# feixh/VISMA

Measured on AMD Instinct MI355X. Metric: icp_iterations_per_sec, higher is better.
Workload: dtype f32; 1 GPU; C4 S-surf 262144->4194304, 4040 ICP iterations of a fresh registration from T=I (cold pass + warm passes), median of 1; ns=262144, nt=4194304, solver=kabsch, nn=grid, search=exact, parallelism=1 GPU, ONE persistent launch per host loop

## Files before the change

### visma_amd/csrc/grid_coop.hip

```cpp
#include <cstdlib>

#include "device_common.h"
#include "grid_coop_probe.h"

namespace visma {

namespace {

struct P12 { float x, y, z; };
#ifndef VISMA_COOP_RU
#define VISMA_COOP_RU 0
#endif
#ifndef VISMA_COOP_CAP
#define VISMA_COOP_CAP (VISMA_COOP_RU ? 344 : 352)
#endif
constexpr bool kCoopRu = VISMA_COOP_RU != 0;
constexpr int kCoopCap = VISMA_COOP_CAP;
#ifndef VISMA_COOP_DEPTH
#define VISMA_COOP_DEPTH 7
#endif
constexpr int kCoopDepth = VISMA_COOP_DEPTH;
#ifndef VISMA_COOP_ROOM
#define VISMA_COOP_ROOM 0.04f
#endif
// ... 7 lines not shown
                 "s_nop 1\n\t"
                 "v_min_f32_dpp %0, %0, %0 quad_perm:[2,3,0,1] row_mask:0xf bank_mask:0xf\n\t"
                 "s_nop 1\n\t"
                 "v_min_f32_dpp %0, %0, %0 row_half_mirror row_mask:0xf bank_mask:0xf"
                 : "=&v"(r)
                 : "v"(d));
    return r;
}

__device__ __forceinline__ unsigned pack_sec(float sec, float third, unsigned lane)
{
    if constexpr (!kCoopRu) return __float_as_uint(sec);
    return (__float_as_uint(sec) & 0xFFFF0000u) | (((__float_as_uint(third) >> 18) & 0x1FFFu) << 3) | (lane & 7u);
}
__device__ __forceinline__ float sec_of(unsigned w) { return __uint_as_float(kCoopRu ? (w & 0xFFFF0000u) : w); }
[[maybe_unused]] __device__ __forceinline__ float third_of(unsigned w) { return __uint_as_float(((w >> 3) & 0x1FFFu) << 18); }

__device__ __forceinline__ unsigned wave_scan_incl(unsigned v, int)
{
    v += (unsigned)__builtin_amdgcn_update_dpp(0, (int)v, 0x111, 0xf, 0xf, false);
    v += (unsigned)__builtin_amdgcn_update_dpp(0, (int)v, 0x112, 0xf, 0xf, false);
    v += (unsigned)__builtin_amdgcn_update_dpp(0, (int)v, 0x114, 0xf, 0xf, false);
    v += (unsigned)__builtin_amdgcn_update_dpp(0, (int)v, 0x118, 0xf, 0xf, false);
    v += (unsigned)__builtin_amdgcn_update_dpp(0, (int)v, 0x142, 0xa, 0xf, false);
    v += (unsigned)__builtin_amdgcn_update_dpp(0, (int)v, 0x143, 0xc, 0xf, false);
    return v;
}

}

struct CoopRes {
    double (*q64)[3];
    float *idx;
    float *lb;
    float *lb3;
    int first;
    double sx, sy, sz;
    int have_src;
};

template <int NTH>
__device__ __forceinline__ void coop_query_range(int ns, int bpp, int lb, int tid, int &vb, int &per_group, long long &i_begin,
                                                 long long &i_end)
{
    vb = lb;
    if ((bpp & 7) == 0) vb = (lb & 7) * (bpp >> 3) + (lb >> 3);
    const int total_groups = bpp * NTH;
    per_group = (ns + total_groups - 1) / total_groups;
    const int gid = vb * NTH + tid;
    i_begin = (long long)gid * per_group;
    i_end = i_begin + per_group < ns ? i_begin + per_group : ns;
}

template <bool PLANE, bool ONE, int NTH, bool PERSIST = false>
__device__ __forceinline__ bool coop_body(
    int ns, const float *__restrict__ s12f, const unsigned *__restrict__ start, GridParams g,
    const float4 *__restrict__ nrm, Xform64 T64, Offset64 off, float r2f, int *__restrict__ idx_out,
    float *__restrict__ d2_out, double *__restrict__ partials, unsigned long long *__restrict__ cand_count,
    const DevIcpState *__restrict__ st, int bpp, long long out_stride, const ProbDesc *__restrict__ descs,
    int nprob, const Pt64 *__restrict__ src64, const Pt64 *__restrict__ sorted64,
    const Pt64 *__restrict__ nrm64, const FoldArgs &fold, double *__restrict__ d64_out,
    Pt64 *__restrict__ wst_io, int warm, Xform64 Tprev, Pt64 *__restrict__ ru_io, unsigned *work_out = nullptr,
    const CoopRes res = CoopRes{})
{
    constexpr int NACC = Acc<PLANE>::N;
    const P12 *s12 = reinterpret_cast<const P12 *>(s12f);
    int prob, lb;
    long long row0;
    if (descs) {
        if (warm & kWarmMap) {
            prob = reinterpret_cast<const int *>(descs + nprob)[blockIdx.x];
        } else {
            int lo = 0, hi = nprob - 1;
            while (lo < hi) {
                const int mid = (lo + hi + 1) >> 1;
                if (descs[mid].first_block <= (int)blockIdx.x) lo = mid; else hi = mid - 1;
            }
            prob = lo;
        }
        const ProbDesc d = descs[prob];
        lb = (int)blockIdx.x - d.first_block;
        bpp = d.nblocks;
        src64 += d.src_off;
        ns = d.ns;
        s12 += d.sorted_off;
        sorted64 += d.sorted_off;
        if constexpr (PLANE) {
            if (nrm) nrm += d.sorted_off;
            if (nrm64) nrm64 += d.sorted_off;
        }
        row0 = d.first_block;
        start += d.start_off;
        g = d.g;
        out_stride = 0;
        idx_out += d.out_off;
        d2_out += d.out_off;
        wst_io += d.out_off;
        if (ru_io) ru_io += d.out_off;
    } else {
        prob = blockIdx.x / bpp;
        lb = blockIdx.x - prob * bpp;
        row0 = (long long)prob * bpp;
    }
    if (st) st += prob;
    {
        Xform32 T32_unused;
        if (!load_loop_state(st, T32_unused, T64, off, r2f)) return false;
        if (st) {
            warm &= ~kWarmTprev;
            if (st->have_prev && !(warm & kWarmNoCert)) {
                warm |= kWarmTprev;
#pragma unroll
                for (int k = 0; k < 12; k++) Tprev.m[k] = st->Tc_prev[k];
            }
        }
        if (!(warm & kWarmRead)) warm &= ~kWarmTprev;
    }
    const double r2d = (double)r2f;
    COOP_PROBE_BEGIN();
    idx_out += (long long)prob * out_stride;
    d2_out += (long long)prob * out_stride;
    wst_io += (long long)prob * out_stride;
    if (ru_io) ru_io += (long long)prob * out_stride;
    double acc[NACC];
#pragma unroll
    for (int a = 0; a < NACC; a++) acc[a] = 0.0;

    const int tid = thread_number<PERSIST, NTH>(), lane = tid & 63, wave = tid >> 6;
    const int oct = lane >> 3, l8 = lane & 7;
    constexpr int NW = NTH / 64;
    constexpr unsigned kCapAll = (unsigned)(NW * kCoopCap);
    int vb, per_group;
    long long i_begin, i_end;
    coop_query_range<NTH>(ns, bpp, lb, tid, vb, per_group, i_begin, i_end);

    __shared__ float4 s_qp[NTH];
    __shared__ uint2 s_item[kCapAll];
    __shared__ unsigned s_sec[kCapAll];
    __shared__ double s_p64[NTH][3];
    __shared__ double s_q64_own[PERSIST ? 1 : NTH][3];
    __shared__ float s_dprev_own[PERSIST ? 1 : NTH];
    double (*s_q64)[3] = s_q64_own;
    float *s_dprev = s_dprev_own;
    if constexpr (PERSIST) { s_q64 = res.q64; s_dprev = res.idx; }
    __shared__ unsigned short s_home[NTH];
    __shared__ unsigned s_need[NW];
    __shared__ unsigned s_m[NW];
    __shared__ unsigned short s_queue[NW][64];

    auto emit = [&](long long i, unsigned ht, bool cert, double bd, unsigned bidx, bool found, double qx, double qy, double qz,
                    float lb_new) {
        if constexpr (PERSIST) {
            res.lb[ht] = lb_new;
            return;
        }
        const unsigned long long lbw = (unsigned long long)__float_as_uint(lb_new) << 32;
        idx_out[i] = found ? (int)bidx : -1;
        if (cert) {
            reinterpret_cast<unsigned *>(&wst_io[i].w)[1] = __float_as_uint(lb_new);
        } else {
            Pt64 o8;
            o8.x = o8.y = o8.z = __longlong_as_double(-1ll);
            o8.w = 0xFFFFFFFFull | lbw;
            if (found) { o8.x = qx; o8.y = qy; o8.z = qz; o8.w = (unsigned long long)bidx | lbw; }
            wst_io[i] = o8;
        }
        d2_out[i] = (float)bd;
        if (d64_out) d64_out[i] = bd;
    };
    auto emit_ru = [&](long long i, unsigned ht, bool have, double ux, double uy, double uz, unsigned uidx, float lb3) {
        if constexpr (kCoopRu) {
            if (!ru_io) return;
            Pt64 o8;
            o8.x = o8.y = o8.z = __longlong_as_double(-1ll);
            o8.w = ~0ull;
            if (have) { o8.x = ux; o8.y = uy; o8.z = uz; o8.w = (unsigned long long)uidx | ((unsigned long long)__float_as_uint(lb3) << 32); }
            ru_io[i] = o8;
            if constexpr (PERSIST) res.lb3[ht] = have ? lb3 : __uint_as_float(0xFFFFFFFFu);
        }
    };
    auto query_p = [&](unsigned h, double (&out)[3]) { out[0] = s_p64[h][0]; out[1] = s_p64[h][1]; out[2] = s_p64[h][2]; };
    auto moments = [&](double pxd, double pyd, double pzd, unsigned bidx, double qx, double qy, double qz) {
        double nx = 0.0, ny = 0.0, nz = 0.0;
        if (PLANE) {
            if (nrm64) { const Pt64 n8 = nrm64[bidx]; nx = n8.x; ny = n8.y; nz = n8.z; }
            else { const float4 n4 = nrm[bidx]; nx = n4.x; ny = n4.y; nz = n4.z; }
        }
        accumulate_pq_d<PLANE>(acc, pxd, pyd, pzd, qx, qy, qz, nx, ny, nz, off);
    };
    auto list_rows = [&](const float px, const float py, const float pz, const float E, const float bound0, const bool want,
                         unsigned (&xb)[9], unsigned (&xe)[9], float &lbgeo2, unsigned &looked) {
        const int cx = cell_coord(px, g.mn[0], g.inv_h, g.dim[0]);
        const int cy = cell_coord(py, g.mn[1], g.inv_hs, g.dim[1]);
        const int cz = cell_coord(pz, g.mn[2], g.inv_hs, g.dim[2]);
        const int x0 = max(cx - 1, 0), x1 = min(cx + 1, g.dim[0] - 1);
        const int span = x1 + 1 - x0;
        typedef unsigned u4a __attribute__((ext_vector_type(4), aligned(4)));
        const bool yok[3] = {cy - 1 >= 0 && cy - 1 < g.dim[1], cy >= 0 && cy < g.dim[1], cy + 1 >= 0 && cy + 1 < g.dim[1]};
        const bool zok[3] = {cz - 1 >= 0 && cz - 1 < g.dim[2], cz >= 0 && cz < g.dim[2], cz + 1 >= 0 && cz + 1 < g.dim[2]};
        const int row_c = (cz * g.dim[1] + cy) * g.dim[0] + x0, pitch_y = g.dim[0], pitch_z = g.dim[1] * g.dim[0];
// ... 152 lines not shown
            if (has_w) {
                const double dx = w8.x - hp[0], dy = w8.y - hp[1], dz = w8.z - hp[2];
                double d = dx * dx;
                d += dy * dy;
                d += dz * dz;
                d2w = d;
                cert = active && t > 0.f && d < r2d && d < (double)t * (double)t * (1.0 - 1e-6);
            } else {
                cert = active && widx == 0xFFFFFFFFu && t > tlim * (1.0f + 1e-6f);
            }
            if (cert) emit(i, (unsigned)tid, true, has_w ? d2w : r2d, widx, has_w, w8.x, w8.y, w8.z, t);
            if constexpr (kCoopRu) {
                const bool has_u = u8.x == u8.x;
                float lb3 = __uint_as_float((unsigned)(u8.w >> 32));
                if constexpr (PERSIST) { if (!res.first) lb3 = res.lb3[tid]; }
                const float t3 = (lb3 - del) * (1.0f - 2.4e-7f);
                if (ru_io && active && has_w && has_u) {
                    if (cert) {
                        if constexpr (PERSIST) res.lb3[tid] = t3;
                        else reinterpret_cast<unsigned *>(&ru_io[i].w)[1] = __float_as_uint(t3);
                    } else if (lb_old > 0.f && t3 > 0.f) {
                        const unsigned uidx = (unsigned)u8.w;
                        const double dx = u8.x - hp[0], dy = u8.y - hp[1], dz = u8.z - hp[2];
                        double d2u = dx * dx;
                        d2u += dy * dy;
                        d2u += dz * dz;
                        const bool u_wins = d2u < d2w || (d2u == d2w && uidx < widx);
                        const double dm = u_wins ? d2u : d2w, dother = u_wins ? d2w : d2u;
                        if (dm < r2d && dm < (double)t3 * (double)t3 * (1.0 - 1e-6)) {
                            cert = true;
                            const float lbn = fminf(t3, sqrtf((float)dother) * (1.0f - 1e-6f));
                            if (u_wins) {
                                const Pt64 ow = w8;
                                w8.x = u8.x; w8.y = u8.y; w8.z = u8.z;
                                w8.w = (unsigned long long)uidx | ((unsigned long long)__float_as_uint(lbn) << 32);
                                widx = uidx;
                                emit_ru(i, (unsigned)tid, true, ow.x, ow.y, ow.z, (unsigned)ow.w, t3);
                                if constexpr (!PERSIST) wst_io[i] = w8;
                            } else {
                                if constexpr (PERSIST) res.lb3[tid] = t3;
                                else reinterpret_cast<unsigned *>(&ru_io[i].w)[1] = __float_as_uint(t3);
                            }
                            emit(i, (unsigned)tid, true, dm, widx, true, w8.x, w8.y, w8.z, lbn);
                        }
                    }
                } else if (ru_io && active && cert) {
                    if constexpr (PERSIST) res.lb3[tid] = __uint_as_float(0xFFFFFFFFu);
                }
            }
        }
        const bool need = active && !cert;
        const bool cfound = cert && has_w;
        s_p64[tid][0] = hp[0]; s_p64[tid][1] = hp[1]; s_p64[tid][2] = hp[2];
        if (need) {
            const float dp = sqdist_f32(make_float4((float)w8.x, (float)w8.y, (float)w8.z, 0.f), (float)hp[0], (float)hp[1], (float)hp[2]);
            const float sq = sqrtf(dp) + kCoopRoom * sqrtf(r2f);
            s_dprev[tid] = sq * sq;
        } else {
            s_q64[tid][0] = w8.x; s_q64[tid][1] = w8.y; s_q64[tid][2] = w8.z;
            s_dprev[tid] = __uint_as_float(cfound ? widx : 0xFFFFFFFFu);
        }
        if (cand_count) {
            const unsigned cc = (unsigned)__builtin_popcountll(__builtin_amdgcn_ballot_w64(cert));
            if (lane == 0 && cc) atomicAdd(cand_count + 2 * 4096 + (blockIdx.x & 4095), (unsigned long long)cc);
        }
        const unsigned long long needers = __builtin_amdgcn_ballot_w64(need);
        const unsigned rank = (unsigned)__builtin_popcountll(needers & ((1ull << lane) - 1ull));
        if (need) s_queue[wave][rank] = (unsigned short)tid;
        if (lane == 0) s_need[wave] = (unsigned)__builtin_popcountll(needers);
        COOP_MARK(9);
        __syncthreads();
        COOP_MARK(10);
        set_phase_prio(1);
        unsigned nq_all = 0;
        unsigned home = 0;
#pragma unroll
        for (int w = 0; w < NW; w++) {
            const unsigned c = (unsigned)__builtin_amdgcn_readfirstlane((int)s_need[w]);
            if ((unsigned)tid >= nq_all && (unsigned)tid < nq_all + c) home = s_queue[w][(unsigned)tid - nq_all];
            nq_all += c;
        }
        const bool searching = (unsigned)(wave * 64) < nq_all;
        const bool sact = (unsigned)tid < nq_all;
        if (nq_all != 0u) {
            unsigned xb[9], xe[9];
            float lbgeo2 = 0.f;
            unsigned nq = 0, off_q = 0;
            if (searching) {
                s_home[tid] = (unsigned short)home;
                double hq[3];
                query_p(home, hq);
                const double pxd = hq[0], pyd = hq[1], pzd = hq[2];
                const float dprev = sact ? s_dprev[home] : __uint_as_float(~0u);
                const float px = (float)pxd, py = (float)pyd, pz = (float)pzd;
                COOP_MARK(0);
                const float rup = sqrtf(r2f) * (1.0f + 2.4e-7f);
                const float E = 2.4e-7f * (fabsf(px) + fabsf(py) + fabsf(pz) + rup) + 4.8e-7f * rup;
                const float tlim = rup + 2.0f * E;
                const float L = tlim * tlim * (1.0f + 6e-7f);
                const float W = (4.0f * E * tlim + 4.0f * E * E) * (1.0f + 1e-6f) + L * 5e-7f;
                s_qp[tid] = make_float4(px, py, pz, W);
                float bound0 = L;
                if (dprev < L) bound0 = dprev;
                unsigned looked;
                list_rows(px, py, pz, E, bound0, sact, xb, xe, lbgeo2, looked);
                asm volatile("" : "+v"(lbgeo2));
                if (cand_count) {
                    unsigned long long c = 0, ca = looked;
#pragma unroll
                    for (int k = 0; k < 9; k++) c += xe[k] - xb[k];
#pragma unroll
                    for (int o = 32; o > 0; o >>= 1) {
                        c += __shfl_down(c, o, 64);
                        ca += __shfl_down(ca, o, 64);
                    }
#ifndef VISMA_COOP_LB_PROBE
                    if (lane == 0 && ca) {
                        unsigned long long *slot = cand_count + 2 * (blockIdx.x & 4095);
                        atomicAdd(slot, c);
                        atomicAdd(slot + 1, ca);
                    }
#endif
                }
                COOP_MARK(1);
#pragma unroll
                for (int k = 0; k < 9; k++) nq += (xe[k] - xb[k] + 7u) >> 3;
                const unsigned incl = wave_scan_incl(nq, lane);
                off_q = incl - nq;
                if (lane == 63) s_m[wave] = incl;
            } else {
                if (lane == 0) s_m[wave] = 0u;
            }
            __syncthreads();
            unsigned m_all = 0;
#pragma unroll
            for (int w = 0; w < NW; w++) {
                const unsigned c = (unsigned)__builtin_amdgcn_readfirstlane((int)s_m[w]);
                if (w < wave) off_q += c;
                m_all += c;
            }
            if (work_out) *work_out = nq_all | (m_all << 12);
            float gh0 = INFINITY, gh1 = INFINITY, gh2 = INFINITY;
            float gsec = INFINITY;
            unsigned gb0 = 0xFFFFFFFFu, gb1 = 0xFFFFFFFFu, gm0 = 0u, gm1 = 0u;
            unsigned gs0 = 0x7F800000u | (0x1FE0u << 3);
            auto chunk_insert = [&](float m, unsigned b, unsigned flags, unsigned side) {
                const bool c1 = m < gh0, c2 = m < gh1;
                gh2 = __builtin_amdgcn_fmed3f(gh1, gh2, m);
                gh1 = __builtin_amdgcn_fmed3f(gh0, gh1, m);
                gh0 = fminf(gh0, m);
                gb1 = c2 ? b : gb1; gm1 = c2 ? flags : gm1;
                gb1 = c1 ? gb0 : gb1; gm1 = c1 ? gm0 : gm1;
                gb0 = c1 ? b : gb0; gm0 = c1 ? flags : gm0;
                if constexpr (kCoopRu) gs0 = c1 ? side : gs0;
            };
            for (unsigned w0 = 0; w0 < m_all; w0 += kCapAll) {
// ... 291 lines not shown
                ru_have = h.x != 0xFFFFFFFFu;
                if (ru_have) ru_pending = sorted64[h.x];
            }
        }
        {
            const unsigned pidx = __float_as_uint(s_dprev[tid]);
            if (active && pidx != 0xFFFFFFFFu) {
                double hq[3];
                query_p((unsigned)tid, hq);
                moments(hq[0], hq[1], hq[2], pidx, s_q64[tid][0], s_q64[tid][1], s_q64[tid][2]);
            }
        }
        if constexpr (!ONE) {
            ru_finish();
            __syncthreads();
        }
    };
    if constexpr (ONE) {
        round(0);
        COOP_MARK(13);
    } else {
        for (int it = 0; it < per_group; it++) round(it);
    }
    COOP_MARK(6);
    COOP_WAVE_DONE();
    bool published = false;
    if constexpr (PERSIST) {
        const unsigned tag = fold_row_tag(fold.seq);
        block_reduce_store<NACC, NW, true>(acc, partials, true, fold.rows_tagged, tag);
        ru_finish();
        COOP_MARK(7);
        published = polled_fold<PLANE, NTH>(fold, lb, bpp, tag);
    } else {
        block_reduce_store<NACC, NW, false>(acc, partials, fold.tickets != nullptr);
        if constexpr (ONE) ru_finish();
        COOP_MARK(7);
        if (fold.tickets) published = fused_fold<PLANE, NTH, false, false>(fold, partials, row0, lb, bpp, prob);
    }
    COOP_MARK(8);
    return published;
}

#define VISMA_COOP_PARAMS                                                                                         \
    int ns, const float *__restrict__ s12f, const unsigned *__restrict__ start, GridParams g,                    \
        const float4 *__restrict__ nrm, Xform64 T64, Offset64 off, float r2f, int *__restrict__ idx_out,         \
        float *__restrict__ d2_out, double *__restrict__ partials, unsigned long long *__restrict__ cand_count,  \
        const DevIcpState *__restrict__ st, int bpp, long long out_stride, const ProbDesc *__restrict__ descs,   \
        int nprob, const Pt64 *__restrict__ src64, const Pt64 *__restrict__ sorted64,                            \
        const Pt64 *__restrict__ nrm64, const FoldArgs fold, double *__restrict__ d64_out,                       \
        Pt64 *__restrict__ wst_io, int warm, Xform64 Tprev, Pt64 *__restrict__ ru_io
#define VISMA_COOP_ARGS                                                                                          \
    ns, s12f, start, g, nrm, T64, off, r2f, idx_out, d2_out, partials, cand_count, st, bpp, out_stride, descs,   \
        nprob, src64, sorted64, nrm64, fold, d64_out, wst_io, warm, Tprev, ru_io
template <bool PLANE>
__global__ __launch_bounds__(kBlock) __attribute__((amdgpu_waves_per_eu(4, 4))) void nn_coop_kernel_one(VISMA_COOP_PARAMS)
{
    (void)coop_body<PLANE, true, kBlock>(VISMA_COOP_ARGS);
}
template <bool PLANE>
__global__ __launch_bounds__(kBlock) void nn_coop_kernel_many(VISMA_COOP_PARAMS)
{
    (void)coop_body<PLANE, false, kBlock>(VISMA_COOP_ARGS);
}

__device__ __forceinline__ unsigned long long persist_wait(const PersistArgs &pa, unsigned tag, bool poller, int pass, int lane)
{
    const bool mine = lane < kPersistWords;
    unsigned long long w = 0ull;
    const bool direct = pa.direct != 0;
    if (poller && lane == 0)
        __hip_atomic_store(pa.relay + kPersistPublished, (unsigned long long)tag, __ATOMIC_RELAXED, __HIP_MEMORY_SCOPE_AGENT);
    long long t_ref = (long long)wall_clock64();
    bool published = poller;
    for (;;) {
        if (mine) {
            if (poller || direct) w = __hip_atomic_load(pa.host_cmd + lane, __ATOMIC_RELAXED, __HIP_MEMORY_SCOPE_SYSTEM);
            else w = __hip_atomic_load(pa.relay + lane, __ATOMIC_RELAXED, __HIP_MEMORY_SCOPE_AGENT);
        }
        const bool ok = !mine || (unsigned)(w >> 32) == tag;
        if (__builtin_amdgcn_ballot_w64(ok) == ~0ull) break;
        const long long now = (long long)wall_clock64();
        bool all_here = true, dead = false;
        if (!published) {
            const unsigned long long m = __hip_atomic_load(pa.relay + kPersistPublished, __ATOMIC_RELAXED, __HIP_MEMORY_SCOPE_AGENT);
            if ((unsigned)m == tag) { published = true; t_ref = now; }
            else {
                all_here = __hip_atomic_load(pa.relay + kPersistStarted, __ATOMIC_RELAXED, __HIP_MEMORY_SCOPE_AGENT) >= (unsigned long long)gridDim.x;
                dead = __hip_atomic_load(pa.relay + kPersistDead, __ATOMIC_RELAXED, __HIP_MEMORY_SCOPE_AGENT) != 0ull;
            }
        }
        const long long limit = published ? pa.wait_ticks : (!all_here ? (pa.start_ticks > 0 ? pa.start_ticks : pa.wait_ticks) : pa.hard_ticks);
        if (dead || now - t_ref > limit) {
            w = ((unsigned long long)tag << 32) | (lane == kPersistWords - 1 ? kPersistAbort : 0u);
            if (lane == 0) {
                __hip_atomic_store(pa.relay + kPersistDead, 1ull, __ATOMIC_RELAXED, __HIP_MEMORY_SCOPE_AGENT);
                __hip_atomic_store(pa.host_flag, (unsigned)pass, __ATOMIC_RELAXED, __HIP_MEMORY_SCOPE_SYSTEM);
            }
            break;
        }
#ifndef VISMA_PERSIST_SLEEP
#define VISMA_PERSIST_SLEEP 1
#endif
        if (poller) __builtin_amdgcn_s_sleep(1); else __builtin_amdgcn_s_sleep(VISMA_PERSIST_SLEEP);
    }
    if (poller && mine && !direct) __hip_atomic_store(pa.relay + lane, w, __ATOMIC_RELAXED, __HIP_MEMORY_SCOPE_AGENT);
    return w;
}

struct CoopPersistParams {
    int ns; const float *s12f; const unsigned *start; GridParams g; const float4 *nrm; Xform64 T64; Offset64 off; float r2f;
    int *idx_out; float *d2_out; double *partials; unsigned long long *cand_count; int bpp; const Pt64 *src64;
    const Pt64 *sorted64; const Pt64 *nrm64; FoldArgs fold; Pt64 *wst_io; int warm; Xform64 Tprev; PersistArgs pa;
    Pt64 *ru_io;
};

template <class T>
__device__ __forceinline__ T ld_karg(const T __attribute__((address_space(4))) *p)
{
    static_assert(sizeof(T) % 4 == 0, "words");
    constexpr int N = (int)(sizeof(T) / 4);
    union U { T v; unsigned w[N]; __device__ U() {} } u;
    typedef const unsigned __attribute__((address_space(4))) *WordPtr;
    const WordPtr pw = (WordPtr)p;
#pragma unroll
    for (int k = 0; k < N; k++) u.w[k] = pw[k];
    return u.v;
}

template <bool PLANE>
__global__ __launch_bounds__(kBlock) __attribute__((amdgpu_waves_per_eu(4, 4))) void nn_coop_kernel_persist(const CoopPersistParams P)
{
    __shared__ unsigned s_tw[2][24];
    __shared__ unsigned s_cmdw;
    __shared__ double r_q64[kBlock][3];
    __shared__ float r_idx[kBlock], r_lb[kBlock], r_lb3[kCoopRu ? kBlock : 1];
    if (threadIdx.x == 0) {
        __hip_atomic_fetch_add(P.pa.relay + kPersistStarted, 1ull, __ATOMIC_RELAXED, __HIP_MEMORY_SCOPE_AGENT);
#pragma unroll
        for (int k = 0; k < 12; k++) {
            const unsigned long long c = (unsigned long long)__double_as_longlong(P.T64.m[k]);
            const unsigned long long q = (unsigned long long)__double_as_longlong(P.Tprev.m[k]);
            s_tw[0][2 * k] = (unsigned)c; s_tw[0][2 * k + 1] = (unsigned)(c >> 32);
            s_tw[1][2 * k] = (unsigned)q; s_tw[1][2 * k + 1] = (unsigned)(q >> 32);
        }
    }
    __syncthreads();
    typedef const CoopPersistParams __attribute__((address_space(4))) *KernargPtr;
#ifndef VISMA_PERSIST_PREFETCH
#define VISMA_PERSIST_PREFETCH 1
#endif
    double nsx = 0.0, nsy = 0.0, nsz = 0.0;
    const int tag_shift = P.pa.wait_first ? 1 : 0;
    if (P.pa.wait_first) {
        const int tidx = thread_number<true>();
        if (tidx < 64) {
            const unsigned long long cw = persist_wait(P.pa, P.pa.tag0, blockIdx.x == 0, 0, tidx);
            if (tidx < 24) s_tw[0][tidx] = (unsigned)cw;
            if (tidx == kPersistWords - 1) s_cmdw = (unsigned)cw;
        }
        __syncthreads();
        if ((unsigned)__builtin_amdgcn_readfirstlane((int)s_cmdw) != kPersistGo) return;
    }
    for (int pass = 1;; pass++) {
        KernargPtr kp = (KernargPtr)__builtin_amdgcn_kernarg_segment_ptr();
        asm volatile("" : "+s"(kp));
#define VISMA_KARG(F_) ld_karg(&kp->F_)
        const unsigned long long t_begin = VISMA_KARG(pa.timeline) ? wall_clock64() : 0ull;
        unsigned work = 0u;
        const int cur = (pass - 1) & 1;
        Xform64 Tc, Tp;
#pragma unroll
        for (int k = 0; k < 12; k++) {
            const unsigned lo = (unsigned)__builtin_amdgcn_readfirstlane((int)s_tw[cur][2 * k]);
            const unsigned hi = (unsigned)__builtin_amdgcn_readfirstlane((int)s_tw[cur][2 * k + 1]);
            Tc.m[k] = __longlong_as_double((long long)(((unsigned long long)hi << 32) | lo));
            Tp.m[k] = 0.0;
        }
        if (pass == 1 || !VISMA_PERSIST_PP_LDS) {
#pragma unroll
            for (int k = 0; k < 12; k++) {
                const unsigned plo = (unsigned)__builtin_amdgcn_readfirstlane((int)s_tw[cur ^ 1][2 * k]);
                const unsigned phi = (unsigned)__builtin_amdgcn_readfirstlane((int)s_tw[cur ^ 1][2 * k + 1]);
                Tp.m[k] = __longlong_as_double((long long)(((unsigned long long)phi << 32) | plo));
            }
        }
        int w = VISMA_KARG(warm);
        if (pass > 1) { w |= kWarmRead; if (!(w & kWarmNoCert)) w |= kWarmTprev; }
        FoldArgs f{};
        f.tickets = VISMA_KARG(fold.tickets); f.partials2 = VISMA_KARG(fold.partials2);
        f.ticket_stride = VISMA_KARG(fold.ticket_stride); f.stats_out = VISMA_KARG(fold.stats_out);
        f.stats_stride = VISMA_KARG(fold.stats_stride); f.host_out = VISMA_KARG(fold.host_out);
        f.seq = VISMA_KARG(fold.seq) + (unsigned long long)(pass - 1);
        f.ipc_n = VISMA_KARG(fold.ipc_n); f.ipc_rank = VISMA_KARG(fold.ipc_rank); f.ipc_seq_dev = VISMA_KARG(fold.ipc_seq_dev);
        f.ipc_flag = VISMA_KARG(fold.ipc_flag); f.ipc_spins = VISMA_KARG(fold.ipc_spins); f.peer_table = VISMA_KARG(fold.peer_table);
        f.rows_tagged = VISMA_KARG(fold.rows_tagged); f.rows2_tagged = VISMA_KARG(fold.rows2_tagged);
        f.dead_flag = VISMA_KARG(fold.dead_flag); f.poll_ticks = VISMA_KARG(fold.poll_ticks);
        const bool published = coop_body<PLANE, true, kBlock, true>(
            VISMA_KARG(ns), VISMA_KARG(s12f), VISMA_KARG(start), VISMA_KARG(g), VISMA_KARG(nrm), Tc, VISMA_KARG(off), VISMA_KARG(r2f),
            VISMA_KARG(idx_out), VISMA_KARG(d2_out), VISMA_KARG(partials), VISMA_KARG(cand_count), nullptr, VISMA_KARG(bpp), 0ll,
            nullptr, 1, VISMA_KARG(src64), VISMA_KARG(sorted64), VISMA_KARG(nrm64), f, nullptr, VISMA_KARG(wst_io), w, Tp,
            VISMA_KARG(ru_io), t_begin ? &work : nullptr, CoopRes{r_q64, r_idx, r_lb, r_lb3, pass == 1 ? 1 : 0, nsx, nsy, nsz,
                                                                        (VISMA_PERSIST_PREFETCH && pass > 1) ? 1 : 0});
        const PersistArgs pa = VISMA_KARG(pa);
        if (pa.timeline && pass <= pa.timeline_passes && thread_number<true>() == 0) {
            unsigned long long *slot = pa.timeline + ((unsigned long long)(pass - 1) * gridDim.x + blockIdx.x) * 2ull;
            slot[0] = t_begin;
            slot[1] = (wall_clock64() & 0xFFFFFFFFFFFull) | ((unsigned long long)work << 44);
        }
        bool last = pass >= pa.max_passes;
        nsx = nsy = nsz = 0.0;
        if (VISMA_PERSIST_PREFETCH && !last) {
            const int tidx = thread_number<true>();
            const int bpp = VISMA_KARG(bpp);
            int vb, per_group;
            long long i_begin, i_end;
            coop_query_range<kBlock>(VISMA_KARG(ns), bpp, (int)blockIdx.x % bpp, tidx, vb, per_group, i_begin, i_end);
            if (i_begin < i_end) {
                const Pt64 s8 = VISMA_KARG(src64)[i_begin];
                nsx = s8.x; nsy = s8.y; nsz = s8.z;
            }
        }
        if (!last) {
            const int tidx = thread_number<true>();
            if (tidx < 64) {
                const bool poller = __builtin_amdgcn_readfirstlane((int)published) != 0;
                const unsigned long long cw = persist_wait(pa, pa.tag0 + (unsigned)(pass - 1 + tag_shift), poller, pass, tidx);
                if (tidx < 24) s_tw[cur ^ 1][tidx] = (unsigned)cw;
                if (tidx == kPersistWords - 1) s_cmdw = (unsigned)cw;
            }
            __syncthreads();
            asm volatile("" : "+v"(nsx), "+v"(nsy), "+v"(nsz));
            const unsigned cmd = (unsigned)__builtin_amdgcn_readfirstlane((int)s_cmdw);
            last = cmd != kPersistGo;
        }
        if (last) {
            const int tidx = thread_number<true>();
            const int bpp = VISMA_KARG(bpp);
            int vb, per_group;
            long long i_begin, i_end;
            coop_query_range<kBlock>(VISMA_KARG(ns), bpp, (int)blockIdx.x % bpp, tidx, vb, per_group, i_begin, i_end);
            if (i_begin < i_end) {
                const unsigned pid = __float_as_uint(r_idx[tidx]);
                Pt64 o8;
                o8.x = r_q64[tidx][0]; o8.y = r_q64[tidx][1]; o8.z = r_q64[tidx][2];
                o8.w = (unsigned long long)pid | ((unsigned long long)__float_as_uint(r_lb[tidx]) << 32);
                float d2 = VISMA_KARG(r2f);
                if (pid != 0xFFFFFFFFu) {
                    double Tl[12];
#pragma unroll
                    for (int k = 0; k < 12; k++)
                        Tl[k] = __longlong_as_double((long long)(((unsigned long long)s_tw[cur][2 * k + 1] << 32) | s_tw[cur][2 * k]));
                    const Pt64 s8 = VISMA_KARG(src64)[i_begin];
                    const double sv[3] = {s8.x, s8.y, s8.z};
                    double hp[3];
                    se3_act(Tl, sv, hp);
                    const double dx = o8.x - hp[0], dy = o8.y - hp[1], dz = o8.z - hp[2];
                    double d = dx * dx;
                    d += dy * dy;
                    d += dz * dz;
                    d2 = (float)d;
                }
                VISMA_KARG(idx_out)[i_begin] = (int)pid;
                VISMA_KARG(d2_out)[i_begin] = d2;
                VISMA_KARG(wst_io)[i_begin] = o8;
                if constexpr (kCoopRu) {
                    Pt64 *ru = VISMA_KARG(ru_io);
                    if (ru) reinterpret_cast<unsigned *>(&ru[i_begin].w)[1] = __float_as_uint(r_lb3[tidx]);
                }
            }
            break;
        }
#undef VISMA_KARG
    }
}
#undef VISMA_COOP_PARAMS
#undef VISMA_COOP_ARGS

#define VISMA_COOP_LAUNCH(KERNEL_)                                                                                  \
    hipLaunchKernelGGL(KERNEL_, dim3(geo.total_blocks), dim3(kBlock), 0, stream, (int)a.ns, a.sorted12, a.start, a.g, \
                       a.nrm, a.T64, a.off, a.r2f, a.idx_out, a.d2_out, a.partials, a.cand_count, a.st, geo.bpp,     \
                       (long long)a.out_stride, a.descs, a.nprob, a.src64, a.sorted64, a.nrm64, a.fold, a.d64_out,   \
                       a.wst_io, warm, Tp, a.ru_io)

hipError_t launch_nn_coop(const SearchArgs &a, const SearchGeom &geo, hipStream_t stream)
{
    if (!a.src64 || !a.sorted64 || !a.sorted12 || !a.wst_io) return hipErrorInvalidValue;
    const FoldArgs &fold = a.fold;
    const int warm = a.Tprev ? (a.warm | kWarmTprev) : (a.warm & ~kWarmTprev);
    if (const PersistArgs *persist = a.persist) {
        if (fold.solve) return hipErrorInvalidValue;
        if (a.descs || a.nprob != 1 || !geo.one || a.st || !fold.rows_tagged || !fold.rows2_tagged || !fold.dead_flag || !fold.host_out ||
            (fold.ipc_n > 1 && !fold.peer_table) || a.d64_out ||
            persist->max_passes < 1 || !persist->host_cmd || !persist->relay || !persist->host_flag ||
            geo.total_blocks > coop_persist_capacity(a.point_to_plane))
            return hipErrorInvalidValue;
        CoopPersistParams P{};
        P.ns = (int)a.ns; P.s12f = a.sorted12; P.start = a.start; P.g = a.g; P.nrm = a.nrm; P.T64 = a.T64; P.off = a.off; P.r2f = a.r2f;
        P.idx_out = a.idx_out; P.d2_out = a.d2_out; P.partials = a.partials; P.cand_count = a.cand_count; P.bpp = geo.bpp;
        P.src64 = a.src64; P.sorted64 = a.sorted64; P.nrm64 = a.nrm64; P.fold = fold; P.wst_io = a.wst_io;
        if (a.Tprev) P.Tprev = *a.Tprev;
        P.warm = warm; P.pa = *persist; P.ru_io = a.ru_io;
        if (a.point_to_plane) hipLaunchKernelGGL(nn_coop_kernel_persist<true>, dim3(geo.total_blocks), dim3(kBlock), 0, stream, P);
        else hipLaunchKernelGGL(nn_coop_kernel_persist<false>, dim3(geo.total_blocks), dim3(kBlock), 0, stream, P);
        return hipGetLastError();
    }
    static const int forced = [] {
        const char *e = std::getenv("VISMA_ICP_COOP_KERNEL");
        return !e ? 0 : (e[0] == 'c' ? 1 : (e[0] == 'w' ? 2 : 0));
    }();
    if (forced == 2 || (forced == 0 && (a.descs || a.nprob > 1))) return launch_nn_wave(a, geo, stream);
    if (fold.solve) return hipErrorInvalidValue;
    Xform64 Tp{};
    if (a.Tprev) Tp = *a.Tprev;
    if (a.point_to_plane) {
        if (geo.one) VISMA_COOP_LAUNCH(nn_coop_kernel_one<true>); else VISMA_COOP_LAUNCH(nn_coop_kernel_many<true>);
    } else {
        if (geo.one) VISMA_COOP_LAUNCH(nn_coop_kernel_one<false>); else VISMA_COOP_LAUNCH(nn_coop_kernel_many<false>);
    }
    return hipGetLastError();
}
#undef VISMA_COOP_LAUNCH

int coop_persist_capacity(int point_to_plane)
{
    static int cap[2][64];
    static bool known[2][64];
    int dev = 0;
    if (hipGetDevice(&dev) != hipSuccess || dev < 0 || dev >= 64) { (void)hipGetLastError(); return 0; }
    const int p = point_to_plane ? 1 : 0;
    if (!known[p][dev]) {
        int per_cu = 0, cus = 0;
        hipError_t e = point_to_plane
                           ? hipOccupancyMaxActiveBlocksPerMultiprocessor(&per_cu, nn_coop_kernel_persist<true>, kBlock, 0)
                           : hipOccupancyMaxActiveBlocksPerMultiprocessor(&per_cu, nn_coop_kernel_persist<false>, kBlock, 0);
        if (e == hipSuccess) e = hipDeviceGetAttribute(&cus, hipDeviceAttributeMultiprocessorCount, dev);
        if (e != hipSuccess) { (void)hipGetLastError(); per_cu = 0; cus = 0; }
        cap[p][dev] = per_cu * cus;
        known[p][dev] = true;
    }
    return cap[p][dev];
}

}
```

### visma_amd/csrc/hip_engine.hpp

```cpp
#pragma once
#include "engine.hpp"

namespace visma {
namespace drv {

class HipEngine : public Engine {
public:
    explicit HipEngine(int device) : device_(device) {}
    ~HipEngine() override
    {
        if (!inited_) { (void)hipGetLastError(); return; }
        (void)hipSetDevice(device_);
        if (sess_live_) (void)end_session();
        if (comm_) g_rccl.CommDestroy(comm_);
        for (int r = 0; r < ipc_n_; r++)
            if (r != ipc_rank_ && peers_.box[r]) (void)hipIpcCloseMemHandle(peers_.box[r]);
        free_dev(d_mbox_); free_dev(d_ipc_flag_); free_dev(d_raw_); free_dev(d_sorted12_); free_dev(bt_sorted12_);
        free_dev(d_pend_count_); free_dev(d_pend_q32_); free_dev(d_pend_q64_); free_dev(d_pend_best_); free_dev(d_pend_idx_);
        for (hipEvent_t e : ev_) (void)hipEventDestroy(e);
        free_dev(d_src_); free_dev(d_tgt_); free_dev(d_nrm_); free_dev(d_keys_); free_dev(d_gkeys_);
        free_dev(d_claim_); free_dev(d_d64_);
        free_dev(d_src64_); free_dev(d_tgt64_); free_dev(d_sorted64_); free_dev(d_nrm64_);
        free_dev(d_snrm_); free_dev(d_snrm64_);
        for (int i = 0; i < 4; i++) if (pin_[i]) (void)hipHostFree(pin_[i]);
// ... 454 lines not shown
    int nn_mode_ = VISMA_ICP_NN_AUTO;
    bool use_grid_ = false, grid_valid_ = false, grid_pending_ = false, brute_reduced_ = false;
    double grid_radius_ = 0.0;
    GridParams grid_{};
    void *d_box_ = nullptr, *d_sorted_ = nullptr, *d_cell_of_ = nullptr, *d_count_ = nullptr;
    void *d_start_ = nullptr, *d_bsum_ = nullptr, *d_cand_ = nullptr;
    void *d_state_ = nullptr;
    DevIcpState *h_state_ = nullptr;
    int state_cap_ = 0;
    size_t partial_rows_ = 0;
    void *bt_src_ = nullptr, *bt_idx_ = nullptr, *bt_d2_ = nullptr, *bt_pos_ = nullptr, *bt_tgt_ = nullptr, *bt_sorted_ = nullptr;
    void *bt_src64_ = nullptr, *bt_tgt64_ = nullptr, *bt_sorted64_ = nullptr;
    int64_t bt_src64_cap_ = 0, bt_tgt64_cap_ = 0;
    void *bt_sorted12_ = nullptr;
    int64_t bt_sorted12_cap_ = 0;
    void *bt_raw_ = nullptr;
    size_t bt_raw_bytes_ = 0;
    void *bt_nrm_ = nullptr, *bt_nrm64_ = nullptr;
    int64_t bt_nrm_cap_ = 0, bt_nrm64_cap_ = 0;
    void *bt_cell_of_ = nullptr, *bt_count_ = nullptr, *bt_start_ = nullptr, *bt_bsum_ = nullptr, *bt_descs_ = nullptr;
    int64_t bt_src_cap_ = 0, bt_tgt_cap_ = 0, bt_cell_cap_ = 0, bt_out_cap_ = 0;
    int bt_bsum_cap_ = 0;
    size_t bt_desc_cap_ = 0;
    std::vector<char> bt_desc_host_;
    int64_t view_offset_ = 0, loop_out_stride_ = 0;
    static constexpr int kGridMaxBlocks = 32768;
    double r2d_ = 0.0;
    bool f64_views() const { return d_src64_ && d_sorted64_; }
    SearchArgs search_args() const
    {
        SearchArgs a;
        a.ns = ns_;
        a.src = (const float4 *)d_src_;
        a.sorted = (const float4 *)d_sorted_;
        if (f64_views()) {
            a.src64 = (const Pt64 *)d_src64_;
            a.sorted64 = (const Pt64 *)d_sorted64_;
            a.sorted12 = (const float *)d_sorted12_;
        }
        a.start = (const unsigned *)d_start_;
        a.g = grid_;
        a.ring = ring_tab_;
        a.nrm = (const float4 *)d_nrm_;
        a.nrm64 = (const Pt64 *)d_nrm64_;
        a.T32 = T32_;
        a.r2f = r2f_;
        a.r2d = r2d_;
        a.exact = exact_ ? 1 : 0;
        a.idx_out = (int32_t *)d_idx_;
        a.d2_out = (float *)d_d2_;
        a.partials = (double *)d_partials_;
        a.wst_io = (Pt64 *)d_pos_;
        a.ru_io = runner_up_ ? (Pt64 *)d_ru_ : nullptr;
        a.warm = kWarmRead;
        return a;
    }
    int grid_sub_ = 1;
    int grid_blocks_env_ = 0;
    int grid_blocks() const
    {
        if (grid_blocks_env_ > 0) return grid_blocks_env_;
        if (grid_.ring > 0) return (int)std::min<int64_t>(kGridMaxBlocks, std::max<int64_t>(1024, (ns_ * (ring_lanes() - 200) + kBlock - 1) / kBlock));
        if (ns_ <= 262144) return 1024;
        return (int)std::min<int64_t>(kGridMaxBlocks, (ns_ + kBlock - 1) / kBlock);
    }
    void *d_pos_ = nullptr;
    bool pos_fresh_ = false;
    void *d_ru_ = nullptr;
    int runner_up_ = 0;
    Xform64 prev_T_{};
    bool prev_T_valid_ = false;
    int cert_enabled_ = 1;
    const Xform64 *cert_prev() const { return (cert_enabled_ && prev_T_valid_ && pos_fresh_) ? &prev_T_ : nullptr; }
    void note_state_pass(const Xform64 &T) { prev_T_ = T; prev_T_valid_ = true; }
    int last_kernel_ = 0;
    int coop_enabled_ = 1;
    int invalidate_pos()
    {
        pos_fresh_ = false;
        prev_T_valid_ = false;
        if (d_pos_ && aux_cap_ > 0) HIP_TRY(hipMemsetAsync(d_pos_, 0xFF, sizeof(Pt64) * (size_t)aux_cap_, stream_));
        if (d_ru_ && aux_cap_ > 0) HIP_TRY(hipMemsetAsync(d_ru_, 0xFF, sizeof(Pt64) * (size_t)aux_cap_, stream_));
        return VISMA_ICP_OK;
    }
    bool coop_ok() const
    {
        return coop_enabled_ && exact_ && d_src64_ && d_sorted64_ && d_sorted12_ && d_pos_ && grid_.sub == 1 && grid_.ring == 0 &&
               (nt_ + kSortedSlack) * 12 < (1ll << 32);
    }
    int pass_kernel(int lanes) const { return grid_.ring > 0 ? 3 : ((lanes == kCoopLanes && coop_ok()) ? 2 : 1); }
    int pass_lanes(int nprob = 1) const
    {
        if (grid_.ring > 0) return ring_lanes();
        if (grid_lanes_ > 0) return grid_lanes_;
        if (coop_ok() && pos_fresh_) return kCoopLanes;
        if (nprob == 1 && cold_in_launch_ && ns_ >= cold_in_launch_min_ns_ && loop_scope_ && loop_budget_ >= 2 && coop_ok() &&
            persist_static_ok())
            return kCoopLanes;
        return grid_lanes(nprob);
    }
    int cold_in_launch_ = 0;
    int64_t cold_in_launch_min_ns_ = 131072;
    int grid_lanes_ = 0;
    int ring_lanes_ = 8;
    bool ring_lanes_auto_ = true;
    double ring_lanes_t84_ = 1.6, ring_lanes_t42_ = 0.8;
    int ring_lanes() const { return 200 + ((ring_lanes_auto_ && !pos_fresh_) ? 8 : ring_lanes_); }
// ... 195 lines not shown
```

### visma_amd/csrc/kernels.h

```cpp
#pragma once

#include <hip/hip_runtime.h>
#include <stdint.h>
#include <vector>

namespace visma {

constexpr int kBlock = 256;
constexpr int kSptLarge = 8;
constexpr int kSptSmall = 2;
constexpr int kSTile = kBlock * kSptLarge;
constexpr int kTChunk = 512;
constexpr int kSub = 64;
constexpr int kReduceAcc = 29;
constexpr int kNStats = 38;

struct Xform32 { float m[12]; };
struct Xform64 { double m[12]; };
struct Offset64 { double v[3]; };
struct Pt64 {
    double x, y, z;
    unsigned long long w;
};

// ... 219 lines not shown
                             int64_t index0 = 0);
hipError_t launch_expand_f32(const float *xyz, int64_t n, int64_t index0, const double c[3], float4 *f4, Pt64 *p8,
                             hipStream_t stream);

hipError_t launch_grid_bbox(const float4 *tgt, int64_t nt, unsigned *box6, hipStream_t stream);
hipError_t launch_pack12(const float4 *src, float *dst, int64_t n, hipStream_t stream);
void grid_decode_bbox(const unsigned box6[6], float mn[3], float mx[3]);
GridParams grid_plan(const float mn[3], const float mx[3], double max_dist, int64_t max_cells, int max_sub = 1);
GridParams grid_plan_ring(const float mn[3], const float mx[3], double max_dist, double cell, int64_t max_cells);
int grid_scan_blocks(int64_t ncell);

hipError_t point_mesh_distance_device(const double *h_P, int64_t np, const double *h_V, int64_t nv,
                                      const int32_t *h_F, int64_t nf, int method, double *h_d2, int32_t *h_face,
                                      double *h_closest, float *kernel_ms, float *build_ms, hipStream_t stream);
hipError_t sample_mesh_transformed_device(const double *h_V, int64_t nv, const int32_t *h_F, int64_t nf, int64_t n,
                                          int quirks, unsigned long long seed, const double *T16, double *d_out,
                                          int64_t room, int64_t *m_out, hipStream_t stream);
hipError_t sample_mesh_device(const double *h_V, int64_t nv, const int32_t *h_F, int64_t nf, int64_t n,
                              int quirks, unsigned long long seed, const double *h_uniforms,
                              double *h_out, int64_t *n_out, hipStream_t stream);
hipError_t surface_distances_device(const double *h_Vs, int64_t nvs, const int32_t *h_Fs, int64_t nfs,
                                    const double *h_Vt, int64_t nvt, const int32_t *h_Ft, int64_t nft, int64_t n,
                                    int quirks, unsigned long long seed, int method, double *h_dist,
                                    int64_t *n_out, float *kernel_ms, float *build_ms, hipStream_t stream);

hipError_t point_cloud_distance_device(const double *h_src, int64_t ns, const double *h_tgt, int64_t nt,
                                       double *h_dist, hipStream_t stream);
hipError_t nearest_neighbor_distance_device(const double *h_xyz, int64_t n, double *h_dist, hipStream_t stream);

constexpr int kNormalsMaxList = 170;
hipError_t estimate_normals_device(const double *h_xyz, int64_t n, const double *h_nrm_in, int search_type,
                                   int knn, double radius, double *h_out, hipStream_t stream);

hipError_t voxel_down_sample_device(const double *h_xyz, const double *h_nrm, const double *h_col,
                                    int64_t n, double voxel, double *h_out_xyz, double *h_out_nrm,
                                    double *h_out_col, int64_t *n_out, hipStream_t stream);
hipError_t voxel_down_sample_core(const double *d_xyz, const double *d_nrm, const double *d_col, int64_t n, double voxel,
                                  double **d_oxyz_out, double **d_onrm_out, double **d_ocol_out, int64_t *n_out,
                                  hipStream_t stream);
hipError_t centroid_device(const double *d_xyz, int64_t n, int64_t chunk, double *d_part, double *d_out, hipStream_t stream);
size_t exclusive_scan_u32_tmp_bytes(long long n);
hipError_t launch_exclusive_scan_u32_lib(const unsigned *in, long long n, unsigned *out, void *tmp, size_t tmp_bytes,
                                         hipStream_t stream);
hipError_t launch_grid_build(const float4 *tgt, int64_t nt, const GridParams &g,
                             unsigned *cell_of, unsigned *count, unsigned *bsum,
                             unsigned *start, float4 *sorted, hipStream_t stream,
                             const Pt64 *tgt64 = nullptr, Pt64 *sorted64 = nullptr);
constexpr int kCoopLanes = 9901;
enum : int {
    kWarmRead = 1,
    kWarmMap = 2,
    kWarmTprev = 4,
    kWarmNoCert = 8,
    kWarmPrioShift = 5, kWarmPrioMask = 3
};
struct SweepArgs {
    unsigned long long *relay;
    unsigned long long *dead;
    int max_passes;
    unsigned tag0;
    int passes0;
    long long wait_ticks;
};

struct SearchArgs {
    int64_t ns = 0;
    const float4 *src = nullptr;
    const Pt64 *src64 = nullptr;
    const float4 *sorted = nullptr;
    const float *sorted12 = nullptr;
    const Pt64 *sorted64 = nullptr;
    const unsigned *start = nullptr;
    GridParams g{};
    RingTable ring{nullptr, 0};
    const float4 *nrm = nullptr;
    const Pt64 *nrm64 = nullptr;
    const ProbDesc *descs = nullptr;
    int nprob = 1;
    int max_blocks = 1;
    int total_blocks = 0;
    int one_per_lane = 0;
    int64_t out_stride = 0;
    Xform32 T32{};
    Xform64 T64{};
    Offset64 off{};
    float r2f = 0.f;
    double r2d = 0.0;
    int point_to_plane = 0;
    int exact = 0;
    int lanes = 0;
    DevIcpState *st = nullptr;
    int warm = 0;
    const Xform64 *Tprev = nullptr;
    FoldArgs fold{};
    const PersistArgs *persist = nullptr;
    int32_t *idx_out = nullptr;
    float *d2_out = nullptr;
    double *d64_out = nullptr;
    double *partials = nullptr;
    unsigned long long *cand_count = nullptr;
    Pt64 *wst_io = nullptr;
    Pt64 *ru_io = nullptr;

    bool packed() const { return src64 != nullptr && exact != 0; }
};
inline int search_blocks(int64_t ns, int lanes, int max_blocks)
// ... 90 lines not shown
```

Measured before the change: 54900 ICP iterations/s.

## Seed cold-pass search bound from home-cell neighbours for stateless queries

Adds a SEED template variant of the cooperative NN kernel. When a query has no prior warm-start state, it first scans its own grid row of up to three cells to get a tentative distance. That distance then tightens the initial search bound before the full exact row listing. The aim is fewer candidate rows in the cold pass, at the cost of an extra cooperative pass with extra barriers, more template instances, and occupancy now capped by the min over both variants.

```diff
diff --git a/visma_amd/csrc/grid_coop.hip b/visma_amd/csrc/grid_coop.hip
--- a/visma_amd/csrc/grid_coop.hip
+++ b/visma_amd/csrc/grid_coop.hip
@@ -83,7 +83,7 @@
     i_end = i_begin + per_group < ns ? i_begin + per_group : ns;
 }
 
-template <bool PLANE, bool ONE, int NTH, bool PERSIST = false>
+template <bool PLANE, bool ONE, int NTH, bool PERSIST = false, bool SEED = false>
 __device__ __forceinline__ bool coop_body(
     int ns, const float *__restrict__ s12f, const unsigned *__restrict__ start, GridParams g,
     const float4 *__restrict__ nrm, Xform64 T64, Offset64 off, float r2f, int *__restrict__ idx_out,
@@ -177,6 +177,7 @@
     __shared__ unsigned short s_home[NTH];
     __shared__ unsigned s_need[NW];
     __shared__ unsigned s_m[NW];
+    __shared__ unsigned s_ms[NW];
     __shared__ unsigned short s_queue[NW][64];
 
     auto emit = [&](long long i, unsigned ht, bool cert, double bd, unsigned bidx, bool found, double qx, double qy, double qz,
@@ -435,10 +436,12 @@
         const bool need = active && !cert;
         const bool cfound = cert && has_w;
         s_p64[tid][0] = hp[0]; s_p64[tid][1] = hp[1]; s_p64[tid][2] = hp[2];
+        bool stateless = false;
         if (need) {
             const float dp = sqdist_f32(make_float4((float)w8.x, (float)w8.y, (float)w8.z, 0.f), (float)hp[0], (float)hp[1], (float)hp[2]);
             const float sq = sqrtf(dp) + kCoopRoom * sqrtf(r2f);
             s_dprev[tid] = sq * sq;
+            if constexpr (SEED) stateless = !(sq == sq) && (unsigned)(w8.w >> 32) == 0xFFFFFFFFu;
         } else {
             s_q64[tid][0] = w8.x; s_q64[tid][1] = w8.y; s_q64[tid][2] = w8.z;
             s_dprev[tid] = __uint_as_float(cfound ? widx : 0xFFFFFFFFu);
@@ -450,22 +453,130 @@
         const unsigned long long needers = __builtin_amdgcn_ballot_w64(need);
         const unsigned rank = (unsigned)__builtin_popcountll(needers & ((1ull << lane) - 1ull));
         if (need) s_queue[wave][rank] = (unsigned short)tid;
-        if (lane == 0) s_need[wave] = (unsigned)__builtin_popcountll(needers);
+        if constexpr (SEED) {
+            const bool any = __builtin_amdgcn_ballot_w64(stateless) != 0ull;
+            if (lane == 0) s_need[wave] = (unsigned)__builtin_popcountll(needers) | (any ? 0x10000u : 0u);
+        } else {
+            if (lane == 0) s_need[wave] = (unsigned)__builtin_popcountll(needers);
+        }
         COOP_MARK(9);
         __syncthreads();
         COOP_MARK(10);
         set_phase_prio(1);
         unsigned nq_all = 0;
         unsigned home = 0;
+        bool seeding = false;
 #pragma unroll
         for (int w = 0; w < NW; w++) {
-            const unsigned c = (unsigned)__builtin_amdgcn_readfirstlane((int)s_need[w]);
+            unsigned c = (unsigned)__builtin_amdgcn_readfirstlane((int)s_need[w]);
+            if constexpr (SEED) {
+                seeding = seeding || (c >> 16) != 0u;
+                c &= 0xFFFFu;
+            }
             if ((unsigned)tid >= nq_all && (unsigned)tid < nq_all + c) home = s_queue[w][(unsigned)tid - nq_all];
             nq_all += c;
         }
         const bool searching = (unsigned)(wave * 64) < nq_all;
         const bool sact = (unsigned)tid < nq_all;
         if (nq_all != 0u) {
+            float seed2 = INFINITY;
+            if (SEED && seeding) {
+                unsigned sb = 0u, se = 0u, nqs = 0u, off_s = 0u;
+                if (searching) {
+                    double hq[3];
+                    query_p(home, hq);
+                    const float px = (float)hq[0], py = (float)hq[1], pz = (float)hq[2];
+                    s_qp[tid] = make_float4(px, py, pz, 0.f);
+                    const float dprev = sact ? s_dprev[home] : 0.f;
+                    const int cx = cell_coord(px, g.mn[0], g.inv_h, g.dim[0]);
+                    const int cy = cell_coord(py, g.mn[1], g.inv_hs, g.dim[1]);
+                    const int cz = cell_coord(pz, g.mn[2], g.inv_hs, g.dim[2]);
+                    const int x0 = max(cx - 1, 0), x1 = min(cx + 1, g.dim[0] - 1);
+                    const int span = x1 + 1 - x0;
+                    if (!(dprev == dprev) && span > 0 && cy >= 0 && cy < g.dim[1] && cz >= 0 && cz < g.dim[2]) {
+                        typedef unsigned u4a __attribute__((ext_vector_type(4), aligned(4)));
+                        const u4a v = *reinterpret_cast<const u4a *>(reinterpret_cast<const char *>(start) + (unsigned)((cz * g.dim[1] + cy) * g.dim[0] + x0) * 4u);
+                        const bool first = cx == x0;
+                        sb = first ? v.x : v.y;
+                        se = first ? v.y : v.z;
+                        if (cx < x0 || cx > x1 || sb == se) {
+                            sb = v.x;
+                            se = span == 3 ? v.w : (span == 2 ? v.z : v.y);
+                        }
+                    }
+                    nqs = (se - sb + 7u) >> 3;
+                    const unsigned incl = wave_scan_incl(nqs, lane);
+                    off_s = incl - nqs;
+                    if (lane == 63) s_ms[wave] = incl;
+                } else {
+                    if (lane == 0) s_ms[wave] = 0u;
+                }
+                __syncthreads();
+                unsigned m_seed = 0;
+#pragma unroll
+                for (int w = 0; w < NW; w++) {
+                    const unsigned c = (unsigned)__builtin_amdgcn_readfirstlane((int)s_ms[w]);
+                    if (w < wave) off_s += c;
+                    m_seed += c;
+                }
+                float sd = INFINITY;
+                for (unsigned w0 = 0; w0 < m_seed; w0 += kCapAll) {
+                    if (searching) {
+                        const unsigned own = (unsigned)tid << 4;
+                        unsigned j = off_s - w0;
+                        for (unsigned b = sb; b < se; b += 8u) {
+                            if (j < kCapAll) s_item[j] = make_uint2(b, own | (min(se - b, 8u) << 16));
+                            j++;
+                        }
+                    }
+                    __syncthreads();
+                    const unsigned mw = min(m_seed - w0, kCapAll);
+                    for (unsigned tb = 0; tb < mw; tb += (unsigned)(NW * 8 * kCoopDepth)) {
+                        const unsigned t = tb + (unsigned)(wave * 8 + oct);
+                        P12 c4[kCoopDepth];
+                        unsigned meta[kCoopDepth];
+#pragma unroll
+                        for (int u = 0; u < kCoopDepth; u++) {
+                            const unsigned c = t + (unsigned)(u * NW * 8);
+                            uint2 dsc = make_uint2(0u, 0u);
+                            if (c < mw) dsc = s_item[c];
+                            meta[u] = dsc.y;
+                            c4[u] = *reinterpret_cast<const P12 *>(reinterpret_cast<const char *>(s12) + (((dsc.x * 3u) << 2) + (unsigned)l8 * 12u));
+                        }
+#pragma unroll
+                        for (int u = 0; u < kCoopDepth; u++) {
+                            const unsigned c = t + (unsigned)(u * NW * 8);
+                            const unsigned cnt = meta[u] >> 16;
+                            const float4 p = *reinterpret_cast<const float4 *>(reinterpret_cast<const char *>(s_qp) + (meta[u] & 0xFFF0u));
+                            float d = sqdist_f32(make_float4(c4[u].x, c4[u].y, c4[u].z, 0.f), p.x, p.y, p.z);
+                            const bool mine = (unsigned)l8 < cnt;
+                            d = mine ? d : INFINITY;
+                            const float m = octet_min(d);
+                            if (l8 == 0 && mine) s_item[c].y = __float_as_uint(m);
+                        }
+                    }
+                    __syncthreads();
+                    if (searching) {
+                        for (unsigned c0 = 0; __builtin_amdgcn_ballot_w64(c0 < nqs) != 0ull; c0 += 4u) {
+                            unsigned r[4];
+                            bool in[4];
+#pragma unroll
+                            for (int u = 0; u < 4; u++) {
+                                const unsigned j = off_s - w0 + c0 + (unsigned)u;
+                                in[u] = c0 + (unsigned)u < nqs && j < kCapAll;
+                                r[u] = s_item[in[u] ? j : 0u].y;
+                            }
+#pragma unroll
+                            for (int u = 0; u < 4; u++) sd = fminf(sd, in[u] ? __uint_as_float(r[u]) : INFINITY);
+                        }
+                    }
+                    if (w0 + kCapAll < m_seed) __syncthreads();
+                }
+                if (sd < INFINITY) {
+                    const float sq = sqrtf(sd) + kCoopRoom * sqrtf(r2f);
+                    seed2 = fmaxf(sq * sq, sd);
+                }
+            }
             unsigned xb[9], xe[9];
             float lbgeo2 = 0.f;
             unsigned nq = 0, off_q = 0;
@@ -485,6 +596,7 @@
                 s_qp[tid] = make_float4(px, py, pz, W);
                 float bound0 = L;
                 if (dprev < L) bound0 = dprev;
+                if constexpr (SEED) { if (seed2 < bound0) bound0 = seed2; }
                 unsigned looked;
                 list_rows(px, py, pz, E, bound0, sact, xb, xe, lbgeo2, looked);
                 asm volatile("" : "+v"(lbgeo2));
@@ -882,15 +994,15 @@
 #define VISMA_COOP_ARGS                                                                                          \
     ns, s12f, start, g, nrm, T64, off, r2f, idx_out, d2_out, partials, cand_count, st, bpp, out_stride, descs,   \
         nprob, src64, sorted64, nrm64, fold, d64_out, wst_io, warm, Tprev, ru_io
-template <bool PLANE>
+template <bool PLANE, bool SEED = false>
 __global__ __launch_bounds__(kBlock) __attribute__((amdgpu_waves_per_eu(4, 4))) void nn_coop_kernel_one(VISMA_COOP_PARAMS)
 {
-    (void)coop_body<PLANE, true, kBlock>(VISMA_COOP_ARGS);
+    (void)coop_body<PLANE, true, kBlock, false, SEED>(VISMA_COOP_ARGS);
 }
-template <bool PLANE>
+template <bool PLANE, bool SEED = false>
 __global__ __launch_bounds__(kBlock) void nn_coop_kernel_many(VISMA_COOP_PARAMS)
 {
-    (void)coop_body<PLANE, false, kBlock>(VISMA_COOP_ARGS);
+    (void)coop_body<PLANE, false, kBlock, false, SEED>(VISMA_COOP_ARGS);
 }
 
 __device__ __forceinline__ unsigned long long persist_wait(const PersistArgs &pa, unsigned tag, bool poller, int pass, int lane)
@@ -957,7 +1069,7 @@
     return u.v;
 }
 
-template <bool PLANE>
+template <bool PLANE, bool SEED = false>
 __global__ __launch_bounds__(kBlock) __attribute__((amdgpu_waves_per_eu(4, 4))) void nn_coop_kernel_persist(const CoopPersistParams P)
 {
     __shared__ unsigned s_tw[2][24];
@@ -1025,7 +1137,7 @@
         f.ipc_flag = VISMA_KARG(fold.ipc_flag); f.ipc_spins = VISMA_KARG(fold.ipc_spins); f.peer_table = VISMA_KARG(fold.peer_table);
         f.rows_tagged = VISMA_KARG(fold.rows_tagged); f.rows2_tagged = VISMA_KARG(fold.rows2_tagged);
         f.dead_flag = VISMA_KARG(fold.dead_flag); f.poll_ticks = VISMA_KARG(fold.poll_ticks);
-        const bool published = coop_body<PLANE, true, kBlock, true>(
+        const bool published = coop_body<PLANE, true, kBlock, true, SEED>(
             VISMA_KARG(ns), VISMA_KARG(s12f), VISMA_KARG(start), VISMA_KARG(g), VISMA_KARG(nrm), Tc, VISMA_KARG(off), VISMA_KARG(r2f),
             VISMA_KARG(idx_out), VISMA_KARG(d2_out), VISMA_KARG(partials), VISMA_KARG(cand_count), nullptr, VISMA_KARG(bpp), 0ll,
             nullptr, 1, VISMA_KARG(src64), VISMA_KARG(sorted64), VISMA_KARG(nrm64), f, nullptr, VISMA_KARG(wst_io), w, Tp,
@@ -1130,8 +1242,14 @@
         P.src64 = a.src64; P.sorted64 = a.sorted64; P.nrm64 = a.nrm64; P.fold = fold; P.wst_io = a.wst_io;
         if (a.Tprev) P.Tprev = *a.Tprev;
         P.warm = warm; P.pa = *persist; P.ru_io = a.ru_io;
-        if (a.point_to_plane) hipLaunchKernelGGL(nn_coop_kernel_persist<true>, dim3(geo.total_blocks), dim3(kBlock), 0, stream, P);
-        else hipLaunchKernelGGL(nn_coop_kernel_persist<false>, dim3(geo.total_blocks), dim3(kBlock), 0, stream, P);
+        const dim3 grid(geo.total_blocks), block(kBlock);
+        if (warm & kWarmSeed) {
+            if (a.point_to_plane) hipLaunchKernelGGL((nn_coop_kernel_persist<true, true>), grid, block, 0, stream, P);
+            else hipLaunchKernelGGL((nn_coop_kernel_persist<false, true>), grid, block, 0, stream, P);
+        } else {
+            if (a.point_to_plane) hipLaunchKernelGGL((nn_coop_kernel_persist<true, false>), grid, block, 0, stream, P);
+            else hipLaunchKernelGGL((nn_coop_kernel_persist<false, false>), grid, block, 0, stream, P);
+        }
         return hipGetLastError();
     }
     static const int forced = [] {
@@ -1142,10 +1260,16 @@
     if (fold.solve) return hipErrorInvalidValue;
     Xform64 Tp{};
     if (a.Tprev) Tp = *a.Tprev;
-    if (a.point_to_plane) {
-        if (geo.one) VISMA_COOP_LAUNCH(nn_coop_kernel_one<true>); else VISMA_COOP_LAUNCH(nn_coop_kernel_many<true>);
+    if (warm & kWarmSeed) {
+        if (a.point_to_plane) {
+            if (geo.one) VISMA_COOP_LAUNCH((nn_coop_kernel_one<true, true>)); else VISMA_COOP_LAUNCH((nn_coop_kernel_many<true, true>));
+        } else {
+            if (geo.one) VISMA_COOP_LAUNCH((nn_coop_kernel_one<false, true>)); else VISMA_COOP_LAUNCH((nn_coop_kernel_many<false, true>));
+        }
+    } else if (a.point_to_plane) {
+        if (geo.one) VISMA_COOP_LAUNCH((nn_coop_kernel_one<true, false>)); else VISMA_COOP_LAUNCH((nn_coop_kernel_many<true, false>));
     } else {
-        if (geo.one) VISMA_COOP_LAUNCH(nn_coop_kernel_one<false>); else VISMA_COOP_LAUNCH(nn_coop_kernel_many<false>);
+        if (geo.one) VISMA_COOP_LAUNCH((nn_coop_kernel_one<false, false>)); else VISMA_COOP_LAUNCH((nn_coop_kernel_many<false, false>));
     }
     return hipGetLastError();
 }
@@ -1160,9 +1284,15 @@
     const int p = point_to_plane ? 1 : 0;
     if (!known[p][dev]) {
         int per_cu = 0, cus = 0;
+        int per_cu_seed = 0;
         hipError_t e = point_to_plane
-                           ? hipOccupancyMaxActiveBlocksPerMultiprocessor(&per_cu, nn_coop_kernel_persist<true>, kBlock, 0)
-                           : hipOccupancyMaxActiveBlocksPerMultiprocessor(&per_cu, nn_coop_kernel_persist<false>, kBlock, 0);
+                           ? hipOccupancyMaxActiveBlocksPerMultiprocessor(&per_cu, nn_coop_kernel_persist<true, false>, kBlock, 0)
+                           : hipOccupancyMaxActiveBlocksPerMultiprocessor(&per_cu, nn_coop_kernel_persist<false, false>, kBlock, 0);
+        if (e == hipSuccess)
+            e = point_to_plane
+                    ? hipOccupancyMaxActiveBlocksPerMultiprocessor(&per_cu_seed, nn_coop_kernel_persist<true, true>, kBlock, 0)
+                    : hipOccupancyMaxActiveBlocksPerMultiprocessor(&per_cu_seed, nn_coop_kernel_persist<false, true>, kBlock, 0);
+        if (e == hipSuccess && per_cu_seed < per_cu) per_cu = per_cu_seed;
         if (e == hipSuccess) e = hipDeviceGetAttribute(&cus, hipDeviceAttributeMultiprocessorCount, dev);
         if (e != hipSuccess) { (void)hipGetLastError(); per_cu = 0; cus = 0; }
         cap[p][dev] = per_cu * cus;
diff --git a/visma_amd/csrc/hip_engine.hpp b/visma_amd/csrc/hip_engine.hpp
--- a/visma_amd/csrc/hip_engine.hpp
+++ b/visma_amd/csrc/hip_engine.hpp
@@ -530,7 +530,7 @@
         a.partials = (double *)d_partials_;
         a.wst_io = (Pt64 *)d_pos_;
         a.ru_io = runner_up_ ? (Pt64 *)d_ru_ : nullptr;
-        a.warm = kWarmRead;
+        a.warm = kWarmRead | (pos_fresh_ ? 0 : kWarmSeed);
         return a;
     }
     int grid_sub_ = 1;
diff --git a/visma_amd/csrc/kernels.h b/visma_amd/csrc/kernels.h
--- a/visma_amd/csrc/kernels.h
+++ b/visma_amd/csrc/kernels.h
@@ -295,6 +295,7 @@
     kWarmMap = 2,
     kWarmTprev = 4,
     kWarmNoCert = 8,
+    kWarmSeed = 16,
     kWarmPrioShift = 5, kWarmPrioMask = 3
 };
 struct SweepArgs {
```

Measured after the change: 55500 ICP iterations/s (median of 4 runs). No clear change (+1.1%).
